# vpc-ccg/tksm

Measured on AMD Instinct MI355X. Metric: sequenced reads/s, higher is better.
Workload: dtype u8; 1 GPU; Bulk molecules, Badread error+qual model (nanopore2020, identity 84,99,5.5), 24 x 128 Mb random genome, FASTQ; kind=bulk, mean_len=1000, length_distribution=normal(1000, 200), compute_qual=True, contexts_in_flight_per_gpu=3

## Files before the change

### __graft_entry__.py

```python
import os
import subprocess
import sys

ROOT = os.path.dirname(os.path.abspath(__file__))


LLVM_BIN = "/opt/rocm/lib/llvm/bin"
NO_SPILL = ("k_alnf", "k_loop", "k_loopw", "k_err", "k_emit", "k_init")
LOOP_VGPR_LIMIT = 128
NO_SPILL_MDF = ("k_noise_plan", "k_noise_fill", "k_pal_count", "k_pal_write",
                "k_mut_count", "k_mut_write")
NO_SPILL_KDE = ("k_kde_grid", "k_kde_sum", "k_kde_cv_min", "k_kde_cv_sum")
NO_SPILL_ABUND = ("k_abund_compat", "k_abund_hits", "k_abund_msum", "k_abund_mfinish", "k_abund_mtotal", "k_abund_estep")
NO_SPILL_MS = ("k_ms_expand", "k_ms_err_events", "k_ms_qs_events")


def kernel_resources(obj):
    import re
    import shutil
    import tempfile
    d = tempfile.mkdtemp(prefix="tksm_co_")
    try:
        tmp = os.path.join(d, os.path.basename(obj))
        shutil.copy(obj, tmp)
        subprocess.check_call([os.path.join(LLVM_BIN, "llvm-objdump"), "--offloading", tmp], stdout=subprocess.DEVNULL)
        cos = [f for f in os.listdir(d) if "amdgcn" in f and "gfx950" in f]
        if not cos:
            raise RuntimeError(f"{obj}: no gfx950 code object inside")
        notes = subprocess.check_output([os.path.join(LLVM_BIN, "llvm-readelf"), "--notes", os.path.join(d, cos[0])], text=True)
    finally:
        shutil.rmtree(d, ignore_errors=True)
    out, cur = {}, None
    for block in notes.split("  - .")[1:]:
        f = dict(re.findall(r"^\s*\.?([a-z_]+):\s+(\S+)\s*$", "." + block, re.M))
        if "name" in f and "vgpr_count" in f:
            out[f["name"]] = {k: int(v) for k, v in f.items() if v.isdigit()}
    return out


def check_no_spills():
    guarded, missing = {}, []
    for obj, names in (("kernels.o", NO_SPILL), ("mdf_kernels.o", NO_SPILL_MDF), ("kde_kernels.o", NO_SPILL_KDE),
                       ("abund_kernels.o", NO_SPILL_ABUND), ("ms_kernels.o", NO_SPILL_MS)):
        res = kernel_resources(os.path.join(ROOT, "tksm_amd", "csrc", "_build", obj))
        found = {n: r for n, r in res.items() if any(f"{len(k)}{k}" in n for k in names)}
        missing += [k for k in names if not any(f"{len(k)}{k}" in n for n in found)]
        guarded.update(found)
    if missing:
        raise RuntimeError(f"spill gate: kernels {missing} not found in the code object (renamed?)")
    bad = {n: r for n, r in guarded.items() if r.get("vgpr_spill_count", 0) or r.get("private_segment_fixed_size", 0)}
    if bad:
        raise RuntimeError("spill gate: scratch spills in " + "; ".join(
            f"{n}: {r.get('vgpr_spill_count')} VGPRs spilled, {r.get('private_segment_fixed_size')} B scratch" for n, r in bad.items()))
    return guarded


def build():
    subprocess.check_call(["make", "-s", "-j8", "-C", os.path.join(ROOT, "tksm_amd", "csrc")])
    guarded = check_no_spills()
    loop = [r for n, r in guarded.items() if "6k_loopE" in n]
    if len(loop) != 1 or loop[0]["vgpr_count"] > LOOP_VGPR_LIMIT:
        raise RuntimeError(f"k_loop: {[r['vgpr_count'] for r in loop]} VGPRs, the limit is {LOOP_VGPR_LIMIT}")
    print(f"k_loop: {loop[0]['vgpr_count']} VGPRs (limit {LOOP_VGPR_LIMIT}), no scratch; LDS per wave 256 B x fragment words per lane "
          f"(at most 64: 16 KB) + the 4 KB bounds table of the first thresholds")
    subprocess.check_call(["make", "-s", "-C", os.path.join(ROOT, "oracle")])
    sys.path.insert(0, ROOT)
    import tksm_amd
    from tksm_amd import _lib
    lib = _lib.load()
    missing = [s for s in _lib.SYMBOLS if not hasattr(lib, s)]
    if missing:
        raise RuntimeError(f"libtksmseq.so lacks symbols: {missing}")


def smoke():
    sys.path.insert(0, ROOT)
    sys.path.insert(0, os.path.join(ROOT, "oracle"))
    import numpy as np
    import pyoracle as po
    from tksm_amd.sequence import Sequencer
    models = os.path.join(ROOT, "tksm_amd", "models", "badread")
    err, qs = os.path.join(models, "nanopore2020.error.gz"), os.path.join(models, "nanopore2020.qscore.gz")
    rs = np.random.RandomState(3)
    ref = {f"c{i}": rs.choice(np.frombuffer(b"ACGT", np.uint8), 50_000).tobytes().decode() for i in range(2)}
    s = Sequencer(0)
    for k, v in ref.items():
        s.add_contig(k, v)
    s.set_identity(84.0, 99.0, 5.5)
    s.load_error_model(err)
    s.load_qscore_model(qs)
    mols = []
    for i in range(16):
        st = int(rs.randint(0, 40_000))
        mols.append((f"m{i}", [(f"c{i % 2}", st, st + 400 + 20 * i, "+-"[i % 2], "3T" if i % 3 == 0 else ""),
                               ("ACGTTTTT", 0, 8, "+", "")]))
    text = "".join(f"+{m}\t1\t\n" + "".join(f"{c}\t{a}\t{b}\t{st}\t{md}\n" for c, a, b, st, md in ivs) for m, ivs in mols)
    b = s.batch_from_mdf(text)
    recs = s.run(b, target="badread", fastq=True, compute_qual=True, seed=9).records()
    perfect = s.run(b, target="perfect", fastq=True, seed=9).records()
    ident = po.Identities(84.0, 5.5, 99.0)
    em, qm = po.ErrorModel(err), po.QScoreModel(qs)
    for i, (mid, ivs) in enumerate(mols):
        raw = po.splice(ref, ivs)
        want, _ = po.badread_record(True, 9, i, raw, ident, em, qm, True, mid)
        assert recs[i] == want, f"badread record {i} differs from the oracle"
        assert perfect[i] == po.perfect_record(True, 9, i, raw, mid), f"perfect record {i} differs from the oracle"
    s.close()
    print("smoke ok: 16 badread + 16 perfect records bit-exact vs the CPU oracle")


if __name__ == "__main__":
    build()
    if len(sys.argv) > 1 and sys.argv[1] == "smoke":
        smoke()
```

### tksm_amd/csrc/ctx.h

```cpp
#pragma once
#include <hip/hip_runtime.h>
#include <chrono>

#include <algorithm>
#include <cstdint>
#include <cstdio>
#include <cstdlib>
#include <map>
#include <memory>
#include <mutex>
#include <string>
#include <unordered_map>
#include <vector>

#include "../../include/tksmseq.h"
#include "abund_kernels.h"
#include "host.h"
#include "kernels.h"
#include "tsb_host.h"

using namespace tkh;

#define HIPCHK(ctx, call)                                                                         \
    do {                                                                                          \
// ... 151 lines not shown
        if (was_owned) release(); else { p = nullptr; cap = 0; }
        p = np; cap = ncap; owned = true; dev = ndev;
        return hipSuccess;
    }
    template <class T> T* as() const { return (T*)p; }
};

struct TmpBuf : DevBuf {
    explicit TmpBuf(hipStream_t s) { pooled = true; pool_stream = s; }
};

struct PinnedBuf {
    void* p = nullptr;
    size_t cap = 0;
    hipError_t ensure(size_t bytes) {
        if (bytes <= cap) return hipSuccess;
        release();
        const hipError_t e = hipHostMalloc(&p, bytes * 2, hipHostMallocDefault);
        if (e != hipSuccess) { p = nullptr; return e; }
        cap = bytes * 2;
        if (Poison::get().on) Poison::get().fill_host(p, cap);
        return hipSuccess;
    }
    void release() { if (p) (void)hipHostFree(p); p = nullptr; cap = 0; }
    ~PinnedBuf() { release(); }
    template <class T> T* as() const { return (T*)p; }
};

struct HelperStream {
    hipStream_t stream = nullptr;
    hipEvent_t start = nullptr, done = nullptr;
    bool used = false;
    hipError_t fork_from(hipStream_t main) {
        hipError_t e = stream ? hipSuccess : hipStreamCreateWithFlags(&stream, hipStreamNonBlocking);
        for (hipEvent_t* ev : {&start, &done}) if (e == hipSuccess && !*ev) e = hipEventCreateWithFlags(ev, hipEventDisableTiming);
        if (e == hipSuccess) e = hipEventRecord(start, main);
        if (e == hipSuccess) e = hipStreamWaitEvent(stream, start, 0);
        return e;
    }
    hipError_t launched() { const hipError_t e = hipEventRecord(done, stream); used = used || e == hipSuccess; return e; }
    hipError_t wait_done() { return hipEventSynchronize(done); }
    hipError_t join_into(hipStream_t main) { return hipStreamWaitEvent(main, done, 0); }
    bool idle() const { return !used || hipEventQuery(done) == hipSuccess; }
    hipError_t synchronize() { return stream ? hipStreamSynchronize(stream) : hipSuccess; }
    ~HelperStream() {
        if (stream) { (void)hipStreamSynchronize(stream); (void)hipStreamDestroy(stream); }
        for (hipEvent_t ev : {start, done}) if (ev) (void)hipEventDestroy(ev);
    }
};

enum RunDiag {
    DIAG_ROUNDS, DIAG_EXACT_KERNEL_READS, DIAG_PREDICTED_STRAGGLERS, DIAG_JOBS_14_ROW_ROUNDS, DIAG_JOBS_REDONE_FULL_WIDTH, DIAG_FALLBACKS,
    DIAG_FALLBACK_REASONS, DIAG_FALLBACKS_QSCORE_JOBS, DIAG_FALLBACKS_LIST_PASS, DIAG_JOBS_ALL_ROUNDS, DIAG_BAND_EXITS,
    DIAG_WORDS = 16
};

struct tksmseq_batch {
    uint64_t n_reads = 0, n_intervals = 0, n_mods = 0, n_literals = 0;
    DevBuf reads, intervals, mods, literals, litpool, ids, idpool;
    tksmseq_batch() { for (DevBuf* b : {&reads, &intervals, &mods, &literals, &litpool, &ids, &idpool, &d_dup, &d_order, &d_tail}) b->pooled = true; }
    std::vector<uint32_t> h_dup;
    DevBuf d_dup;
    std::vector<uint32_t> h_comments;
    std::vector<char> h_comment_pool;
    std::vector<uint32_t> raw_len;
    std::vector<uint32_t> order;
    DevBuf d_order;
    uint32_t max_raw = 0;
    uint64_t total_raw = 0;
    std::vector<uint32_t> splice_len;
    DevBuf d_tail;
    bool tail_on = false;
    uint64_t tail_key[4] = {};
    int cache_k = -1, cache_num = 0, cache_den = 0, cache_add = 0;
    uint64_t cache_scratch = 0;
};

struct tksmseq_ctx : ContigLookup {
    int device = 0;
    int n_cus = 256;
    hipStream_t stream = nullptr;
    static constexpr int N_SIDE = 4, SIDE_WAVES = 512;
    HelperStream side[N_SIDE];
    HelperStream early;
    uint32_t early_tail = 1024;
    DevBuf f_early;
    bool own_stream = false;
    std::string err;

    std::vector<std::string> contig_names;
    std::unordered_map<std::string, int> contig_index;
    std::vector<uint64_t> contigs;
    uint64_t total_alloc = 0;
    uint64_t total_bases = 0;
    uint32_t pool_blocks = 0;
    std::vector<uint8_t> contig_declared; uint32_t n_declared = 0;
    uint64_t ref_version = 0, wgs_version = ~0ull;
    DevBuf d_wgs_sofar, d_wgs_nameoff, d_wgs_namelen, d_wgs_names;
    DevBuf d_packed, d_blocktab, d_pool, d_contigs, d_stage;
    std::shared_ptr<const tsb::Transcripts> tsb;
    uint64_t tsb_dev_serial = 0, tsb_ref_version = ~0ull;
    DevBuf d_tsb_first, d_tsb_exons, d_tsb_lits, d_tsb_litpool;
    uint64_t tsb_n_lits = 0, tsb_lit_bytes = 0;
    float tsb_plan_ms = 0.f, tsb_write_ms = 0.f;
    uint64_t mut_serial = 0, mut_ref_version = ~0ull;
    DevBuf d_mut_refctg, d_mut_nameoff, d_mut_names, d_mut_delfirst, d_mut_ptfirst, d_mut_delfrom, d_mut_delto, d_mut_ptpos, d_mut_ptinfo, d_mut_insent, d_mut_inspool;
// ... 62 lines not shown
```

### tksm_amd/csrc/kernels.h

```cpp
#pragma once
#include <hip/hip_runtime.h>
#include <stdint.h>

namespace tk {

constexpr uint32_t NO_BLOCK = 0xFFFFFFFFu;
constexpr int BLOCK_SHIFT = 12;
constexpr int WAVES_PER_WG = 4;

struct RefView {
    const uint32_t* packed;
    const uint32_t* blocktab;
    const uint8_t* pool;
    const uint64_t* contigs;
    uint32_t n_contigs;
};

struct BatchView {
    const uint32_t* reads;
    const uint32_t* intervals;
    const uint32_t* mods;
    const uint64_t* literals;
    const uint8_t* litpool;
    const uint32_t* ids;
// ... 72 lines not shown
    unsigned long long* work_counter;
    int32_t* istats;
    double* dstats;
    uint8_t* full_pool; unsigned long long full_pool_bytes; unsigned long long* full_pool_used;
    const uint32_t* tail_len;
    const TailChain* tail_chain;
    uint8_t* big_scratch; size_t big_per_wave; unsigned long long* big_trace;
    const uint32_t* read_list;
    uint64_t n_work;
};

struct ReadState {
    double errors, target, est;
    int32_t change_count;
    uint32_t n_base, aln_no;
    int16_t resume_src, resume_j;
    uint8_t stage;
    uint8_t pending, slow, early;
    int32_t st_draws, st_aligns;
    uint32_t job;
    int32_t raw_len;
    uint32_t res_mt, res_cols, res_fail, pad3;
};

struct RangeGeo {
    uint64_t trace_off;
    uint64_t jc_off;
    uint64_t popd_off;
    uint64_t unused;
    uint32_t tstride;
    uint32_t cw;
    uint32_t ncap;
    uint32_t pad;
};

enum Counter {
    CNT_JOBS = 0,
    CNT_DEFERRED = 1,
    CNT_SLOW = 2,
    CNT_FULL_ROWS = 3,
    CNT_EXIT = 4,
    CNT_REDO_JOBS = 8,
    CNT_REDO_WAVES = 9,
    CNT_REDO_LIST = 10,
    CNT_FAIL = 12,
    CNT_FAIL_OR = 13,
    CNT_FAIL_LAST = 14,
    CNT_FAIL_NM = 15,
    CNT_FAIL_REASON = 16,
    CNT_FAIL_QJOB = 24,
    CNT_FAIL_LIST = 25,
    CNT_EARLY_SLOW = 26,
    CNT_EARLY = 27,
    CNT_WORDS = 32
};
enum ExitCause { EXIT_BAND_LOOP = 0, EXIT_SHIFT_LOOP = 1, EXIT_SHIFT_ERR = 2, EXIT_BAND_ERR = 3 };
enum FailBit { FAIL_QUEUE = 0, FAIL_NOROW = 1, FAIL_SHIFT31 = 3, FAIL_SHIFT14 = 4, FAIL_END_CELL = 5, FAIL_WALK = 6 };

struct FastBuffers {
    ReadState* state;
    const uint32_t* row64;
    uint8_t* st_frag;
    uint16_t* st_nb;
    unsigned long long* st_fplanes;
    uint32_t* st_frag2;
    uint32_t* job_meta;
    uint8_t* job_popd;
    void* trace;
    uint32_t* redo_list;
    void* trace_full;
    uint32_t full_rows, full_tg;
    uint32_t full_cl;
    uint32_t* counters;
    uint32_t* job_cnt;
    uint32_t rs, n_ranges;
    const uint32_t* prev_meta; const uint8_t* prev_popd;
    const uint32_t* prefix;
    const uint32_t* base_cur; const uint32_t* base_prev;
    const RangeGeo* geo_cur; const RangeGeo* geo_prev;
    uint32_t* slow_list;
    uint32_t* early_hist;
    uint2* early_list;
    uint32_t* early_slow;
    uint2* defer_list;
    uint32_t* defer_cnt;
    int defer_len;
};

hipError_t launch_pack(const uint8_t* ascii, uint64_t n, uint64_t gstart, uint32_t* packed, uint32_t* blockflag,
                       hipStream_t s);
hipError_t launch_fill_pool(const uint8_t* ascii, uint64_t n, uint64_t gstart, const uint32_t* blocktab,
                            uint8_t* pool, hipStream_t s);
hipError_t launch_read_lengths(const BatchView& b, const RefView& r, int k, int cap_num, int cap_den, int cap_add,
                               const uint32_t* tail_len, uint32_t* raw_len, uint64_t* slot_cap, uint32_t* status, hipStream_t s);
hipError_t launch_tail_lengths(const BatchView& B, const RefView& R, const TailView& T, uint64_t seed, uint64_t first_read,
                               uint64_t stride, uint32_t* tail_len, hipStream_t s);
hipError_t launch_simulate(const BatchView& b, const RefView& r, const ErrModelView& em, const QsModelView& qm,
                           const IdentView& im, const SimParams& p, const SimBuffers& o, int n_wgs,
                           int waves_per_wg, hipStream_t s);
size_t simulate_big_bytes(int lcap, int ncap);
hipError_t launch_simulate_big(const BatchView& b, const RefView& r, const ErrModelView& em, const QsModelView& qm,
                               const IdentView& im, const SimParams& p, const SimBuffers& o, int n_waves, hipStream_t s);
hipError_t launch_init(const BatchView& b, const RefView& r, const ErrModelView& em, const IdentView& im, const SimParams& p,
                       const SimBuffers& o, const FastBuffers& fb, int waves_per_wg, hipStream_t s);
int err_lds_bytes(int lcap, int ncap, int waves_per_wg, bool state_in_hbm);
int loop_lds_words(int lcap);
// ... 34 lines not shown
```

### tksm_amd/csrc/kernels.hip

```cpp
#include "kernels.h"
#include "loop_filter.h"
#include <type_traits>

namespace tk {

#define DEV __device__ __forceinline__

constexpr int BIG = 1 << 28;
DEV bool is_inf(int v) { return v >= (1 << 27); }

struct Ph4 { uint32_t x, y, z, w; };
enum { ST_ID = 0, ST_PAD = 1, ST_IDENT = 2, ST_DRAW = 3, ST_ALNPOS = 4, ST_QUAL = 5, ST_TAIL = 6 };

DEV Ph4 philox(uint64_t seed, uint64_t read, uint32_t stream, uint32_t n) {
    uint32_t c0 = (uint32_t)read, c1 = (uint32_t)(read >> 32), c2 = stream, c3 = n;
    uint32_t k0 = (uint32_t)seed, k1 = (uint32_t)(seed >> 32);
#pragma unroll
    for (int r = 0; r < 10; r++) {
        const unsigned long long p0 = (unsigned long long)0xD2511F53u * c0, p1 = (unsigned long long)0xCD9E8D57u * c2;
        const uint32_t h0 = (uint32_t)(p0 >> 32), l0 = (uint32_t)p0, h1 = (uint32_t)(p1 >> 32), l1 = (uint32_t)p1;
        uint32_t n0 = h1 ^ c1 ^ k0, n2 = h0 ^ c3 ^ k1;
        c0 = n0; c1 = l1; c2 = n2; c3 = l0;
        k0 += 0x9E3779B9u; k1 += 0xBB67AE85u;
    }
    return Ph4{c0, c1, c2, c3};
}

DEV uint8_t base_char(int code) { return (uint8_t)((0x54474341u >> (8 * (code & 3))) & 0xff); }
DEV int code_of(uint8_t c) { return c == 'A' ? 0 : c == 'C' ? 1 : c == 'G' ? 2 : c == 'T' ? 3 : -1; }
DEV uint8_t upper(uint8_t c) { return (c >= 'a' && c <= 'z') ? (uint8_t)(c - 32) : c; }
DEV uint8_t comp(uint8_t c) {
    return c == 'A' ? 'T' : c == 'C' ? 'G' : c == 'G' ? 'C' : c == 'T' ? 'A' : c;
}

template <int CTRL, int ROW_MASK> DEV int dpp_mov(int old, int src) { return __builtin_amdgcn_update_dpp(old, src, CTRL, ROW_MASK, 0xf, false); }
constexpr int DPP_WAVE_SHL1 = 0x130, DPP_WAVE_SHR1 = 0x138;
#define TKSM_DPP_SCAN(OP, IDENT, x)                         \
    x = OP(x, dpp_mov<0x111, 0xf>(IDENT, x));               \
    x = OP(x, dpp_mov<0x112, 0xf>(IDENT, x));               \
    x = OP(x, dpp_mov<0x114, 0xf>(IDENT, x));               \
    x = OP(x, dpp_mov<0x118, 0xf>(IDENT, x));               \
    x = OP(x, dpp_mov<0x142, 0xa>(IDENT, x));               \
    x = OP(x, dpp_mov<0x143, 0xc>(IDENT, x));
DEV int scan_min_incl(int x, int) { TKSM_DPP_SCAN(min, 0x7fffffff, x) return x; }
DEV int scan_max_incl(int x, int) { TKSM_DPP_SCAN(max, (int)0x80000000, x) return x; }
DEV int add_i32(int a, int b) { return a + b; }
DEV int scan_add_incl(int x, int) { TKSM_DPP_SCAN(add_i32, 0, x) return x; }
DEV uint32_t scan_umax_incl(uint32_t x) {
#define TKSM_UMAX_STEP(C, R) x = max(x, (uint32_t)dpp_mov<C, R>(0, (int)x));
    TKSM_UMAX_STEP(0x111, 0xf) TKSM_UMAX_STEP(0x112, 0xf) TKSM_UMAX_STEP(0x114, 0xf) TKSM_UMAX_STEP(0x118, 0xf) TKSM_UMAX_STEP(0x142, 0xa) TKSM_UMAX_STEP(0x143, 0xc)
#undef TKSM_UMAX_STEP
    return x;
}
DEV int prefix_small(int v, int& total) {
// ... 1610 lines not shown
        uint32_t lo2 = c0, hi2 = c1 - 1;
        while (lo2 < hi2) { const uint32_t mid = (lo2 + hi2 + 1) >> 1; if (FB.prefix[mid] <= target) lo2 = mid; else hi2 = mid - 1; }
        const uint32_t pjob = FB.base_prev[lo2] + (target - FB.prefix[lo2]);
        r = (uint64_t)__builtin_amdgcn_readfirstlane((int)FB.prev_meta[4ull * pjob]) & 0xffffffffull;
        pos = lo2 * FB.rs;
    }
    ReadState S = FB.state[r];
    if (S.stage == 2 || S.slow) return;
    if (S.stage == 0) return;
    uint16_t* gnb = nb_row(FB, r);
    const int per_wave = STATE_IN_HBM ? lds_ncap + 128 : lds_lcap * 3 + lds_ncap + 128;
    uint8_t* lds_wave = lds_raw + (size_t)wave * per_wave;
    uint8_t* frag = STATE_IN_HBM ? frag_row(FB, r) : lds_wave;
    uint16_t* nb = STATE_IN_HBM ? gnb : reinterpret_cast<uint16_t*>(lds_wave + lds_lcap);
    uint8_t* aux = STATE_IN_HBM ? lds_wave : lds_wave + 3 * (size_t)lds_lcap;
    const int k = EM.k;
    const uint64_t g = P.first_read + r * P.stride;
    const int raw_len = __builtin_amdgcn_readfirstlane(S.raw_len);
    const int L = raw_len + 2 * k;
    const uint64_t slot = O.slot_off[r];
    const int cap = __builtin_amdgcn_readfirstlane((int)((O.slot_off[r + 1] - slot) >> 1));
    uint8_t* out_seq = O.scratch + slot;
    uint8_t* out_qual = out_seq + cap;
    if (!STATE_IN_HBM) {
        const uint8_t* gfrag0 = frag_row(FB, r);
        for (int t = lane * 4; t < L; t += 256) *reinterpret_cast<uint32_t*>(frag + t) = *reinterpret_cast<const uint32_t*>(gfrag0 + t);
        for (int t = lane * 2; t < L; t += 128) *reinterpret_cast<uint32_t*>(nb + t) = *reinterpret_cast<const uint32_t*>(gnb + t);
    }
    wave_sync();
    uint32_t status = 0;
    const double frag_len = (double)L;
    const double errors = S.errors;
    const double target = S.target;
    const int change_count = __builtin_amdgcn_readfirstlane(S.change_count), st_draws = __builtin_amdgcn_readfirstlane(S.st_draws);
    int st_aligns = __builtin_amdgcn_readfirstlane(S.st_aligns);
    double identity = 1.0;

    int start_trim, end_trim;
    {
        int v1 = lane < k ? slot_len(nb[lane]) : 0, v2 = lane < k ? slot_len(nb[L - k + lane]) : 0;
        (void)prefix_small(v1, start_trim);
        (void)prefix_small(v2, end_trim);
    }
    const int jcap = min(lds_ncap, cap);
    const int m = joined_len(nb, 0, L, lane);
    int lo = start_trim, hi = end_trim == 0 ? 0 : m - end_trim;
    lo = min(lo, m); hi = max(hi, lo);
    if (m > jcap) { status |= 1; lo = hi = 0; }
    const int out_len = hi - lo;
    const bool want_q = P.compute_q && m > 0 && !(status & 1);
    if (want_q) {
        const uint32_t mt = S.res_mt, cols = S.res_cols, fail = S.res_fail;
        if (fail) { go_slow(FB, r, lane, EXIT_BAND_ERR); return; }
        identity = cols ? (double)mt / (double)cols : 0.0;
        const uint32_t rc1 = pos / FB.rs;
        const uint8_t* gp = FB.prev_popd + FB.geo_prev[rc1].popd_off + (size_t)(S.job - FB.base_prev[rc1]) * FB.geo_prev[rc1].ncap;
        wave_sync();
        uint8_t* popd = aux + 16;
        for (int t = lane; t < m; t += 64) popd[t] = gp[t];
        wave_sync();
        const int margins = (QM.kmer_size - 1) / 2;
        const uint32_t hmask = (uint32_t)QM.n_slots - 1u;
        for (int i2 = lo + lane; i2 < hi; i2 += 64) {
#ifdef TKSM_ABLATE
            if (P.ablate == 40) { out_qual[i2 - lo] = 40; continue; }
#endif
            const int d = max(0, max(margins - i2, i2 + margins - (m - 1)));
            int row = -1; uint32_t roff = 0, rcnt = 0;
            auto probe = [&](uint64_t key) {
                uint32_t sl = (uint32_t)qs_hash(key) & hmask;
#ifdef TKSM_ABLATE
                if (P.ablate == 41) { row = (int)(sl & 1023u); roff = 0u; rcnt = 1u; return; }
#endif
                for (;;) {
                    const uint4 e = QM.ent[sl];
                    const uint64_t kk = ((uint64_t)e.y << 32) | e.x;
                    if (kk == key) { row = (int)sl; roff = e.z; rcnt = e.w; break; }
                    if (kk == 0) break;
                    sl = (sl + 1) & hmask;
                }
            };
            if (margins <= 4) {
                const int ob = 16 + i2 - 4, sh = ob & 3;
                const uint32_t* aw = reinterpret_cast<const uint32_t*>(aux) + (ob >> 2);
                const uint32_t w0 = aw[0], w1 = aw[1], w2 = aw[2];
                const uint32_t b0 = __builtin_amdgcn_alignbyte(w1, w0, sh), b1 = __builtin_amdgcn_alignbyte(w2, w1, sh), b2 = w2 >> (8 * sh);
                auto byte_at = [&](int j) -> uint32_t { return j < 4 ? (b0 >> (8 * j)) & 255u : j < 8 ? (b1 >> (8 * (j - 4))) & 255u : b2 & 255u; };
                uint64_t K[5]; int ln[5];
                K[0] = byte_at(4) & 3u; ln[0] = 1;
#pragma unroll
                for (int h = 1; h <= 4; h++) {
                    const uint32_t bl = byte_at(4 - h);
                    const int ddl = (int)(bl >> 2), ddr = (int)(byte_at(3 + h) >> 2);
                    ln[h] = ln[h - 1] + 2 + ddl + ddr;
                    const bool fits = ln[h] <= 29;
                    const int sl_ = fits ? 2 * (1 + ddl) : 0, sr_ = fits ? 2 * (1 + ddl + ln[h - 1]) : 0, so_ = fits ? 2 * (ln[h] - 1) : 0;
                    const int dl2 = fits ? 2 * ddl : 0, dr2 = fits ? 2 * ddr : 0;
                    K[h] = (uint64_t)(bl & 3u) | (((1ull << dl2) - 1ull) << 2) | (K[h - 1] << sl_) | (((1ull << dr2) - 1ull) << sr_) |
                           ((uint64_t)(byte_at(4 + h) & 3u) << so_);
                }
                const int hmax = margins - d;
                bool pend = true;
#pragma unroll
                for (int h = 4; h >= 0; h--) {
                    const bool tryit = pend && h <= hmax;
                    if (__ballot(tryit) == 0ull) continue;
                    if (tryit && ln[h] <= 29) { probe(K[h] | ((uint64_t)ln[h] << 58)); pend = row < 0; }
#ifdef TKSM_ABLATE
                    if (P.ablate == 44) { if (row < 0) row = (int)(K[h] & 1023u); pend = false; }
                    if (P.ablate == 45 && h == 3) { if (row < 0) row = (int)(K[h] & 1023u); pend = false; }
#endif
                }
            } else {
                int s0 = i2 - margins + d, e0 = i2 + margins - d;
                for (;;) {
                    uint64_t key = 0; int len = 0; bool ok = true;
                    for (int x2 = s0; x2 <= e0; x2++) {
                        if (x2 > s0) {
                            const int dd = popd[x2 - 1] >> 2;
                            if (len + dd > 29) { ok = false; break; }
                            key |= ((1ull << (2 * dd)) - 1ull) << (2 * len); len += dd;
                        }
                        if (len >= 29) { ok = false; break; }
                        key |= (uint64_t)(popd[x2] & 3) << (2 * len); len++;
                    }
                    if (ok) probe(key | ((uint64_t)len << 58));
                    if (row >= 0 || s0 == e0) break;
                    s0++; e0--;
                }
            }
            uint8_t q = 0;
#ifdef TKSM_ABLATE
            if (P.ablate == 42) { out_qual[i2 - lo] = (uint8_t)(33 + (row & 31)); continue; }
            if (P.ablate == 43 && row >= 0) {
                const uint32_t w = (uint32_t)i2 * 2654435761u;
                const uint32_t a2 = QM.guide[(size_t)row * 64 + (w >> 26)] & 0x7fu;
                out_qual[i2 - lo] = (uint8_t)(33 + QM.pairs[roff + min(a2, rcnt - 1u)].y); continue;
            }
#endif
            if (row >= 0) {
                const uint32_t w = philox(P.seed, g, ST_QUAL, (uint32_t)i2).x;
                uint32_t a2 = QM.guide[(size_t)row * 64 + (w >> 26)];
                if (QM.guide_direct && (a2 & 0x80u)) q = (uint8_t)(a2 & 0x7fu);
                else {
                    uint2 pr = QM.pairs[roff + a2];
                    while (a2 + 1 < rcnt && !(w < pr.x)) { a2++; pr = QM.pairs[roff + a2]; }
                    q = (uint8_t)pr.y;
                }
            }
            out_qual[i2 - lo] = (uint8_t)(q + 33);
        }
    } else {
        identity = 1.0 - errors / frag_len;
    }
    join_out(frag, nb, L, out_seq, lo, hi, lane);
    if (P.quirk_perfect) identity = 1.0;
    finish_read(B, P, O, r, P.quirk_perfect ? out_len : raw_len, out_len, identity, status, st_draws, change_count, st_aligns, L, m,
                start_trim, end_trim, errors, target, lane);
    if (lane == 0) FB.state[r].stage = 2;
}

__global__ void k_collect_unfinished(FastBuffers FB, uint64_t n_reads) {
    const uint64_t r = (uint64_t)blockIdx.x * blockDim.x + threadIdx.x;
    if (r >= n_reads) return;
    ReadState S = FB.state[r];
    if (S.stage != 2 && !S.slow) {
        FB.state[r].slow = 1;
        const uint32_t idx = atomicAdd(&FB.counters[CNT_SLOW], 1u);
        FB.slow_list[idx] = (uint32_t)r;
    }
}

DEV uint32_t range_of_job(const FastBuffers& FB, uint32_t job0) {
    uint32_t rng = 0, hi2 = FB.n_ranges - 1;
    while (rng < hi2) { const uint32_t mid = (rng + hi2 + 1) >> 1; if (FB.base_cur[mid] <= job0) rng = mid; else hi2 = mid - 1; }
    return rng;
}
__global__ __launch_bounds__(64) void k_qjobs(FastBuffers FB, int k, uint32_t count) {
    const int lane = threadIdx.x;
    const uint32_t widx = blockIdx.x * 64u + (uint32_t)lane;
    bool need = widx < count;
    uint32_t r = 0, rc = 0, job = 0;
    if (need) { const uint2 e = FB.defer_list[widx]; r = e.x; rc = e.y; }
    need = need && FB.state[r].stage == 3 && !FB.state[r].slow;
    const bool mine = need;
    unsigned long long todo = __ballot(need);
    while (todo) {
        const int leader = __builtin_ctzll(todo);
        const uint32_t lrc = (uint32_t)__shfl((int)rc, leader, 64);
        const unsigned long long grp = __ballot(need && rc == lrc);
        uint32_t base = 0;
        if (lane == leader) base = FB.base_cur[lrc] + atomicAdd(&FB.job_cnt[lrc * 32u], (uint32_t)__popcll(grp));
        base = (uint32_t)__shfl((int)base, leader, 64);
        if (need && rc == lrc) { job = base + (uint32_t)__popcll(grp & ((1ull << lane) - 1ull)); need = false; }
        todo &= ~grp;
    }
    if (mine) {
        ReadState* sp = FB.state + r;
        const uint32_t L = (uint32_t)(sp->raw_len + 2 * k);
        *reinterpret_cast<uint4*>(FB.job_meta + 4ull * job) = make_uint4(r, 0u, L | 0x80000000u, 0u);
        sp->resume_src = -1; sp->pending = 1; sp->stage = 1; sp->job = job;
    }
}

DEV int wave_max(int v) {
#pragma unroll
    for (int o = 32; o > 0; o >>= 1) v = max(v, __shfl_xor(v, o, 64));
    return v;
// ... 1009 lines not shown
```

### tksm_amd/csrc/run.cpp

```cpp
#include "../../include/tksmseq.h"

#include <hip/hip_runtime.h>

#include <algorithm>
#include <cstdio>
#include <cstring>
#include <cstdlib>
#include <string>

#include "ctx.h"

#define TRY(call) do { const int rc_ = (call); if (rc_ != TKSMSEQ_OK) return rc_; } while (0)

static tk::BatchView batch_view(const tksmseq_batch* b) {
    return tk::BatchView{b->reads.as<uint32_t>(), b->intervals.as<uint32_t>(), b->mods.as<uint32_t>(), b->literals.as<uint64_t>(),
                         b->litpool.as<uint8_t>(), b->ids.as<uint32_t>(), b->idpool.as<uint8_t>(), b->n_reads, (uint32_t)b->n_literals};
}
static tk::RefView ref_view(const tksmseq_ctx* ctx) {
    return tk::RefView{ctx->d_packed.as<uint32_t>(), ctx->d_blocktab.as<uint32_t>(), ctx->d_pool.as<uint8_t>(),
                       ctx->d_contigs.as<uint64_t>(), (uint32_t)ctx->contig_names.size()};
}

static int apply_tail(tksmseq_ctx* ctx, tksmseq_batch* b, const tksmseq_run_params* p) {
    const bool want = p->mode == TKSMSEQ_MODE_BADREAD && ctx->tail.enabled && b->n_reads > 0;
// ... 408 lines not shown
    int align(bool qround) {
        const uint32_t jobs = cnt[tk::CNT_JOBS];
        const uint32_t n_jobs = hbase_cur[FB.n_ranges - 1] + ((hcnt[(size_t)(FB.n_ranges - 1) * 32] + 63) & ~63u);
        const bool full_only = jobs <= std::min(ctx->small_aln, full_rows_fit);
        jobs_all += jobs; if (!full_only) jobs_14 += jobs;
        HIPCHK(ctx, tk::launch_alnf(pl.P, FB, pl.O, n_jobs, full_only, qround ? 1 : 0, s));
        return tick(ALN);
    }
    int rounds() {
        for (;; n_rounds++) {
            select_set(n_rounds);
            HIPCHK(ctx, tk::launch_round_reset(FB, s));
            TRY(tick(GAP));
            const bool qround = revive && pl.P.compute_q;
            const bool regular = !revive && !revived;
            TRY(revive ? launch_revive() : revived ? launch_last_visits() : launch_loops());
            TRY(tick(regular ? JOB : OTHER));
            TRY(exchange());
            TRY(flush_side());
            if (cnt[tk::CNT_JOBS] == 0) {
                TRY(join_early());
                if (cnt[tk::CNT_DEFERRED] == 0 || revived) break;
                revived = revive = true; n_deferred = cnt[tk::CNT_DEFERRED];
                std::vector<uint32_t> hd((size_t)FB.n_ranges * 32);
                HIPCHK(ctx, hipMemcpy(hd.data(), ctx->f_defercnt.p, hd.size() * 4, hipMemcpyDeviceToHost));
                HIPCHK(ctx, pack_ranges(hd.data(), true));
                continue;
            }
#ifdef TKSM_ABLATE
            if (pl.P.ablate >= 1 && pl.P.ablate <= 9) break;
#endif
            if (cnt[tk::CNT_JOBS] < ctx->tail_cut && cnt[tk::CNT_JOBS] * 64ull < n) {
                HIPCHK(ctx, tk::launch_collect_unfinished(FB, n, s));
                HIPCHK(ctx, hipMemcpyAsync(cnt, FB.counters, 64, hipMemcpyDeviceToHost, s));
                HIPCHK(ctx, hipStreamSynchronize(s));
                break;
            }
            if (n_rounds > 100000) { ctx->err = "internal: error loop did not terminate"; return TKSMSEQ_EDEVICE; }
            TRY(tick(GAP));
            TRY(align(qround));
            HIPCHK(ctx, pack_ranges(hcnt, false));
        }
        pl.mark("rounds done");
        return TKSMSEQ_OK;
    }
    int finish(float ms[3]) {
        uint32_t* d = ctx->last_diag;
        memset(d, 0, sizeof(ctx->last_diag));
        d[DIAG_ROUNDS] = n_rounds; d[DIAG_EXACT_KERNEL_READS] = cnt[tk::CNT_SLOW]; d[DIAG_PREDICTED_STRAGGLERS] = n_early;
        d[DIAG_JOBS_14_ROW_ROUNDS] = (uint32_t)std::min<uint64_t>(jobs_14, 0xffffffffu); d[DIAG_JOBS_REDONE_FULL_WIDTH] = cnt[tk::CNT_REDO_JOBS];
        d[DIAG_FALLBACKS] = cnt[tk::CNT_FAIL]; d[DIAG_FALLBACK_REASONS] = cnt[tk::CNT_FAIL_OR]; d[DIAG_FALLBACKS_QSCORE_JOBS] = cnt[tk::CNT_FAIL_QJOB];
        d[DIAG_FALLBACKS_LIST_PASS] = cnt[tk::CNT_FAIL_LIST]; d[DIAG_JOBS_ALL_ROUNDS] = (uint32_t)std::min<uint64_t>(jobs_all, 0xffffffffu);
        d[DIAG_BAND_EXITS] = cnt[tk::CNT_EXIT + tk::EXIT_BAND_LOOP] + cnt[tk::CNT_EXIT + tk::EXIT_BAND_ERR];
        if (pl.vlevel) {
            uint32_t cc[tk::CNT_WORDS];
            HIPCHK(ctx, hipMemcpy(cc, FB.counters, sizeof(cc), hipMemcpyDeviceToHost));
            const uint32_t *ex = cc + tk::CNT_EXIT, *why = cc + tk::CNT_FAIL_REASON;
            fprintf(stderr, "[tksmseq] this thread so far: %u device allocations, %.3f s in hipMalloc\n", alloc_calls(), alloc_seconds());
            fprintf(stderr, "[tksmseq] reads %llu rounds %u slow-path reads %u (band exit %u/%u, shift %u/%u), full-width redo: %u jobs in %u waves; predicted stragglers on their own stream: %u\n",
                    (unsigned long long)n, n_rounds, cnt[tk::CNT_SLOW], ex[tk::EXIT_BAND_LOOP], ex[tk::EXIT_BAND_ERR], ex[tk::EXIT_SHIFT_LOOP], ex[tk::EXIT_SHIFT_ERR], cc[tk::CNT_REDO_JOBS], cc[tk::CNT_REDO_WAVES], n_early);
            fprintf(stderr, "[tksmseq] fused alignment failures: %u, reasons or-ed 0x%x, last 0x%x (n %u, m %u)\n", cc[tk::CNT_FAIL], cc[tk::CNT_FAIL_OR], cc[tk::CNT_FAIL_LAST], cc[tk::CNT_FAIL_NM] & 0xffffu, cc[tk::CNT_FAIL_NM] >> 16);
            fprintf(stderr, "[tksmseq]   per reason: queue / reservoir overflow %u no pool rows %u - shift>31 %u shift>14 %u end cell %u walk %u | q-score jobs %u, list pass %u\n", why[tk::FAIL_QUEUE], why[tk::FAIL_NOROW], why[tk::FAIL_SHIFT31], why[tk::FAIL_SHIFT14], why[tk::FAIL_END_CELL], why[tk::FAIL_WALK], cc[tk::CNT_FAIL_QJOB], cc[tk::CNT_FAIL_LIST]);
        }
        for (HelperStream& h : ctx->side) if (h.used) HIPCHK(ctx, h.join_into(s));
        if (cnt[tk::CNT_SLOW] > n_side) {
            pl.O.read_list = ctx->f_slow.as<uint32_t>() + n_side; pl.O.n_work = cnt[tk::CNT_SLOW] - n_side;
            const uint64_t want = (pl.O.n_work + pl.wpw - 1) / pl.wpw;
            TRY(tick(GAP));
            HIPCHK(ctx, tk::launch_simulate(pl.B, pl.R, pl.EM, pl.QM, pl.IM, pl.P, pl.O, (int)std::max<uint64_t>(1, std::min<uint64_t>(want, (uint64_t)pl.n_wgs)), pl.wpw, s));
            TRY(tick(OTHER));
        }
        if (ctx->timing) {
            HIPCHK(ctx, hipStreamSynchronize(s));
            for (size_t i = 1; i < kinds.size(); i++) {
                float t = 0; (void)hipEventElapsedTime(&t, ctx->evpool[i - 1], ctx->evpool[i]);
                if (kinds[i] >= LOOP) ms[kinds[i] - LOOP] += t;
            }
        }
        return TKSMSEQ_OK;
    }
};

static int rerun_in_hbm(const RunPlan& pl, const std::vector<uint32_t>& st) {
    tksmseq_ctx* ctx = pl.ctx;
    hipStream_t s = ctx->stream;
    std::vector<uint32_t> big;
    for (uint64_t i = 0; i < pl.n; i++) if (st[i] & 8) big.push_back((uint32_t)i);
    const int n_waves = (int)std::min<size_t>(big.size(), 64);
    const size_t per_wave = tk::simulate_big_bytes(pl.lcap, pl.ncap);
    HIPCHK(ctx, ctx->w_biglist.ensure(big.size() * 4 + 16));
    HIPCHK(ctx, ctx->w_bigscratch.ensure(per_wave * n_waves + 64));
    HIPCHK(ctx, ctx->w_bigtrace.ensure((size_t)n_waves * 2 * (pl.ncap + 2) * 8 + 64));
    HIPCHK(ctx, hipMemcpyAsync(ctx->w_biglist.p, big.data(), big.size() * 4, hipMemcpyHostToDevice, s));
    HIPCHK(ctx, hipMemsetAsync(ctx->w_counter.p, 0, 8, s));
    tk::SimBuffers O3 = pl.O;
    O3.read_list = ctx->w_biglist.as<uint32_t>(); O3.n_work = big.size();
    O3.work_counter = ctx->w_counter.as<unsigned long long>();
    O3.big_scratch = ctx->w_bigscratch.as<uint8_t>(); O3.big_per_wave = per_wave; O3.big_trace = ctx->w_bigtrace.as<unsigned long long>();
    HIPCHK(ctx, tk::launch_simulate_big(pl.B, pl.R, pl.EM, pl.QM, pl.IM, pl.P, O3, n_waves, s));
    if (pl.vlevel) fprintf(stderr, "[tksmseq] %zu molecules beyond the LDS-resident limit took the exact kernel with HBM working sets\n", big.size());
    return TKSMSEQ_OK;
}

static int check_status(const RunPlan& pl, int pass, bool* again, bool* overflow) {
    tksmseq_ctx* ctx = pl.ctx;
    const uint64_t n = pl.n;
// ... 131 lines not shown
```

### tksm_amd/sequence.py

```python
import ctypes as C

import numpy as np

from . import _lib as L

BGZF_EOF = bytes.fromhex("1f8b08040000000000ff0600424302001b0003000000000000000000")


class TksmSeqError(RuntimeError):
    def __init__(self, code, msg):
        super().__init__(f"tksmseq error {code}: {msg}")
        self.code = code


class Batch:
    def __init__(self, seq, handle):
        self._seq, self._h = seq, handle
        n, ni, nm = C.c_uint64(), C.c_uint64(), C.c_uint64()
        seq._lib.tksmseq_batch_info(handle, C.byref(n), C.byref(ni), C.byref(nm))
        self.n_reads, self.n_intervals, self.n_mods = n.value, ni.value, nm.value

    def free(self):
        if self._h:
            self._seq._lib.tksmseq_batch_free(self._seq._ctx, self._h)
# ... 514 lines not shown
        t, n = C.c_void_p(), C.c_uint64()
        self._chk(self._lib.tksmseq_batch_to_mdf_text(self._ctx, batch._h, C.byref(t), C.byref(n)))
        try:
            return C.string_at(t, n.value).decode()
        finally:
            self._lib.tksmseq_text_free(t)

    def run(self, batch, target="badread", fastq=True, compute_qual=True, seed=42, first_read_index=0, stride=1,
            collect_stats=False, perfect_of_badread=False):
        p = L.RunParams(seed, first_read_index, stride, L.MODE_BADREAD if target == "badread" else L.MODE_PERFECT,
                        1 if fastq else 0, 1 if compute_qual else 0, 1 if collect_stats else 0,
                        1 if perfect_of_badread else 0, 0)
        r = L.Result()
        self._chk(self._lib.tksmseq_run(self._ctx, batch._h, C.byref(p), C.byref(r)))
        return RunResult(self, r)

    def mdf_to_seq(self, molecules, target="perfect", **kw):
        lines = []
        for mid, intervals in molecules:
            lines.append(f"+{mid}\t1\t\n")
            for chrom, start, end, strand, mods in intervals:
                lines.append(f"{chrom}\t{start}\t{end}\t{strand}\t{mods}\n")
        b = self.batch_from_mdf("".join(lines))
        try:
            return self.run(b, target=target, **kw).records()
        finally:
            b.free()

    def _gzip_fetch(self, g, with_info):
        out = np.empty(g.bytes, np.uint8)
        self._chk(self._lib.tksmseq_gzip_download_range(self._ctx, out.ctypes.data, 0, g.bytes, 0))
        if not with_info:
            return out.tobytes()
        off = np.empty(g.n_members + 1, np.uint64)
        self._chk(self._lib.tksmseq_gzip_download_offsets(self._ctx, off.ctypes.data))
        return out.tobytes(), off, g.device_ms

    def gzip_device(self, ptr, nbytes, format=L.GZIP_RAW, with_info=False):
        fmt = {"raw": L.GZIP_RAW, "fasta": L.GZIP_FASTA, "fastq": L.GZIP_FASTQ}.get(format, format)
        g = L.GzipResult()
        self._chk(self._lib.tksmseq_gzip_device(self._ctx, C.c_void_p(ptr) if ptr else None, nbytes, fmt, C.byref(g)))
        return self._gzip_fetch(g, with_info)

    def set_host_threads(self, n):
        self._chk(self._lib.tksmseq_set_host_threads(self._ctx, int(n)))

    def set_timing(self, on=True):
        self._chk(self._lib.tksmseq_set_timing(self._ctx, 1 if on else 0))

    def run_diagnostics(self):
        out = (C.c_uint32 * 16)()
        self._chk(self._lib.tksmseq_run_diagnostics(self._ctx, out))
        keys = ("rounds", "exact_kernel_reads", "predicted_stragglers", "jobs_14_row_rounds", "jobs_redone_full_width", "fallbacks",
                "fallback_reasons", "fallbacks_qscore_jobs", "fallbacks_list_pass", "jobs_all_rounds", "band_exits")
        return {k: int(out[i]) for i, k in enumerate(keys)}

    def set_output_buffer(self, ptr, capacity):
        self._chk(self._lib.tksmseq_set_output_buffer(self._ctx, C.c_void_p(ptr) if ptr else None, capacity))

    def synchronize(self):
        self._chk(self._lib.tksmseq_synchronize(self._ctx))

    def interleave_records(self, streams, offsets, n_per_rank, dst_ptr, dst_capacity):
        n = len(streams)
        sp = (C.c_void_p * n)(*[C.c_void_p(s) for s in streams])
        op = (C.c_void_p * n)(*[C.c_void_p(o) for o in offsets])
        npr = (C.c_uint64 * n)(*n_per_rank)
        out = C.c_uint64()
        self._chk(self._lib.tksmseq_interleave_records(self._ctx, n, sp, op, npr, C.c_void_p(dst_ptr), dst_capacity,
                                                       C.byref(out)))
        return out.value


def random_wgs_main(argv):
    lib = L.load()
    arr = (C.c_char_p * len(argv))(*[a.encode() for a in argv])
    return lib.tksmseq_random_wgs_main(len(argv), arr)


def transcribe_main(argv):
    lib = L.load()
    arr = (C.c_char_p * len(argv))(*[a.encode() for a in argv])
    return lib.tksmseq_transcribe_main(len(argv), arr)


def sequence_main(argv):
    lib = L.load()
    arr = (C.c_char_p * len(argv))(*[a.encode() for a in argv])
    return lib.tksmseq_sequence_main(len(argv), arr)


def build_tail_model(mapped, unmapped, lx, ly, begin, trans, bandwidth, path, device=0):
    import json
    mapped = np.asarray(mapped, np.float64).ravel(); unmapped = np.asarray(unmapped, np.float64).ravel()
    lx = np.asarray(lx, np.float64).ravel(); ly = np.asarray(ly, np.float64).ravel()
    trans = np.asarray(trans, np.float64); begin = np.asarray(begin, np.float64).ravel()
    if len(mapped) != len(unmapped) or len(mapped) == 0:
        raise ValueError("tail model: mapped and unmapped must be non-empty and of one length")
    if len(lx) != len(ly):
        raise ValueError("tail model: lx and ly must have the same length (the reference's sampler reads grid rows by ly)")
    if trans.shape != (4, 4) or begin.shape != (4,):
        raise ValueError("tail model: begin must hold 4 weights, trans 4 x 4")
    s = Sequencer(device)
    try:
        grid = s.kde_grid(np.stack([mapped, unmapped], axis=1), lx, ly, bandwidth)
    finally:
        s.close()
# ... 6 lines not shown
```

Measured before the change: 15.66 million reads/s.

## Build qscore k-mer keys from a packed LDS op stream with prefix offsets

For the quality-score pass, each wave now packs the alignment op sequence into a 2-bit token stream in LDS, using a wave prefix scan for offsets. Each position's centred window key for sizes 4..1 then becomes a single bit-slice of that stream, replacing the per-position byte-walk key construction. The old per-position path is kept as a fallback when the stream does not fit in LDS or the state lives in HBM. The change also moves join_out ahead of the quality pass and adds diagnostic counters, which cost extra atomics in the hot loop.

```diff
diff --git a/__graft_entry__.py b/__graft_entry__.py
--- a/__graft_entry__.py
+++ b/__graft_entry__.py
@@ -8,6 +8,7 @@
 LLVM_BIN = "/opt/rocm/lib/llvm/bin"
 NO_SPILL = ("k_alnf", "k_loop", "k_loopw", "k_err", "k_emit", "k_init")
 LOOP_VGPR_LIMIT = 128
+ERR_VGPR_LIMIT = 64
 NO_SPILL_MDF = ("k_noise_plan", "k_noise_fill", "k_pal_count", "k_pal_write",
                 "k_mut_count", "k_mut_write")
 NO_SPILL_KDE = ("k_kde_grid", "k_kde_sum", "k_kde_cv_min", "k_kde_cv_sum")
@@ -63,6 +64,10 @@
         raise RuntimeError(f"k_loop: {[r['vgpr_count'] for r in loop]} VGPRs, the limit is {LOOP_VGPR_LIMIT}")
     print(f"k_loop: {loop[0]['vgpr_count']} VGPRs (limit {LOOP_VGPR_LIMIT}), no scratch; LDS per wave 256 B x fragment words per lane "
           f"(at most 64: 16 KB) + the 4 KB bounds table of the first thresholds")
+    err = {("<true>" if "ILb1E" in n else "<false>"): r["vgpr_count"] for n, r in guarded.items() if "5k_errI" in n}
+    if len(err) != 2 or max(err.values()) > ERR_VGPR_LIMIT:
+        raise RuntimeError(f"k_err: {err} VGPRs, the limit is {ERR_VGPR_LIMIT}")
+    print(f"k_err: {err['<false>']} / {err['<true>']} VGPRs (state in LDS / in HBM; limit {ERR_VGPR_LIMIT}), no scratch")
     subprocess.check_call(["make", "-s", "-C", os.path.join(ROOT, "oracle")])
     sys.path.insert(0, ROOT)
     import tksm_amd
diff --git a/tksm_amd/csrc/ctx.h b/tksm_amd/csrc/ctx.h
--- a/tksm_amd/csrc/ctx.h
+++ b/tksm_amd/csrc/ctx.h
@@ -227,6 +227,7 @@
 enum RunDiag {
     DIAG_ROUNDS, DIAG_EXACT_KERNEL_READS, DIAG_PREDICTED_STRAGGLERS, DIAG_JOBS_14_ROW_ROUNDS, DIAG_JOBS_REDONE_FULL_WIDTH, DIAG_FALLBACKS,
     DIAG_FALLBACK_REASONS, DIAG_FALLBACKS_QSCORE_JOBS, DIAG_FALLBACKS_LIST_PASS, DIAG_JOBS_ALL_ROUNDS, DIAG_BAND_EXITS,
+    DIAG_QS_KEYS_PER_POSITION, DIAG_QS_GAPS_29, DIAG_QS_WINDOWS_29, DIAG_QS_WINDOWS_30,
     DIAG_WORDS = 16
 };
 
diff --git a/tksm_amd/csrc/kernels.h b/tksm_amd/csrc/kernels.h
--- a/tksm_amd/csrc/kernels.h
+++ b/tksm_amd/csrc/kernels.h
@@ -148,6 +148,10 @@
     CNT_FAIL_LIST = 25,
     CNT_EARLY_SLOW = 26,
     CNT_EARLY = 27,
+    CNT_QS_PERPOS = 28,
+    CNT_QS_GAP29 = 29,
+    CNT_QS_LEN29 = 30,
+    CNT_QS_LEN30 = 31,
     CNT_WORDS = 32
 };
 enum ExitCause { EXIT_BAND_LOOP = 0, EXIT_SHIFT_LOOP = 1, EXIT_SHIFT_ERR = 2, EXIT_BAND_ERR = 3 };
diff --git a/tksm_amd/csrc/kernels.hip b/tksm_amd/csrc/kernels.hip
--- a/tksm_amd/csrc/kernels.hip
+++ b/tksm_amd/csrc/kernels.hip
@@ -1,5 +1,6 @@
 #include "kernels.h"
 #include "loop_filter.h"
+#include "qs_keys.h"
 #include <type_traits>
 
 namespace tk {
@@ -1716,6 +1717,7 @@
     if (want_q) {
         const uint32_t mt = S.res_mt, cols = S.res_cols, fail = S.res_fail;
         if (fail) { go_slow(FB, r, lane, EXIT_BAND_ERR); return; }
+        join_out(frag, nb, L, out_seq, lo, hi, lane);
         identity = cols ? (double)mt / (double)cols : 0.0;
         const uint32_t rc1 = pos / FB.rs;
         const uint8_t* gp = FB.prev_popd + FB.geo_prev[rc1].popd_off + (size_t)(S.job - FB.base_prev[rc1]) * FB.geo_prev[rc1].ncap;
@@ -1725,25 +1727,98 @@
         wave_sync();
         const int margins = (QM.kmer_size - 1) / 2;
         const uint32_t hmask = (uint32_t)QM.n_slots - 1u;
+        int row = -1; uint32_t roff = 0, rcnt = 0;
+        auto probe = [&](uint64_t key) {
+            uint32_t sl = (uint32_t)qs_hash(key) & hmask;
+#ifdef TKSM_ABLATE
+            if (P.ablate == 41) { row = (int)(sl & 1023u); roff = 0u; rcnt = 1u; return; }
+#endif
+            for (;;) {
+                const uint4 e = QM.ent[sl];
+                const uint64_t kk = ((uint64_t)e.y << 32) | e.x;
+                if (kk == key) { row = (int)sl; roff = e.z; rcnt = e.w; break; }
+                if (kk == 0) break;
+                sl = (sl + 1) & hmask;
+            }
+        };
+        auto draw_q = [&](int i2) {
+            uint8_t q = 0;
+            if (row >= 0) {
+                const uint32_t w = philox(P.seed, g, ST_QUAL, (uint32_t)i2).x;
+                uint32_t a2 = QM.guide[(size_t)row * 64 + (w >> 26)];
+                if (QM.guide_direct && (a2 & 0x80u)) q = (uint8_t)(a2 & 0x7fu);
+                else {
+                    uint2 pr = QM.pairs[roff + a2];
+                    while (a2 + 1 < rcnt && !(w < pr.x)) { a2++; pr = QM.pairs[roff + a2]; }
+                    q = (uint8_t)pr.y;
+                }
+            }
+            out_qual[i2 - lo] = (uint8_t)(q + 33);
+        };
+        bool use_stream = false;
+        const uint32_t nw = tkqk::qs_stream_words(cols);
+        if constexpr (!STATE_IN_HBM) use_stream = margins <= 4 && cols >= (uint32_t)m && cols < 65536u && (int)(nw * 4u) + 2 * m <= 3 * lds_lcap;
+#ifdef TKSM_ABLATE
+        if (P.ablate >= 40 && P.ablate <= 46) use_stream = false;
+#endif
+        if constexpr (!STATE_IN_HBM) { if (!use_stream && margins <= 4 && lane == 0) atomicAdd(&FB.counters[CNT_QS_PERPOS], 1u); }
+        if (use_stream) {
+            uint32_t* strm = reinterpret_cast<uint32_t*>(lds_wave);
+            uint16_t* offs = reinterpret_cast<uint16_t*>(strm + nw);
+            for (uint32_t t = (uint32_t)lane; t < nw; t += 64) strm[t] = 0u;
+            wave_sync();
+            int base = 0;
+            for (int xb = 0; xb < m; xb += 64) {
+                const int x = xb + lane;
+                const uint32_t b = x < m ? popd[x] : 0u;
+                const int tl = x < m ? tkqk::qs_token_units(b) : 0;
+                const int incl = scan_add_incl(tl, lane);
+                const int off = base + incl - tl;
+                base += __builtin_amdgcn_readlane(incl, 63);
+                if (x < m) offs[x] = (uint16_t)off;
+                if (x < m && (b >> 2) >= (uint32_t)tkqk::QS_GAP_MAX) atomicAdd(&FB.counters[CNT_QS_GAP29], 1u);
+                const uint64_t tok = x < m ? tkqk::qs_token(b) : 0ull;
+                if (tok) {
+                    const uint32_t w = (uint32_t)off >> 4, sh = (2u * (uint32_t)off) & 31u;
+                    const uint32_t t0 = lo32(tok) << sh, t1 = sh ? alignbit(hi32(tok), lo32(tok), 32u - sh) : hi32(tok);
+                    const uint32_t t2 = sh ? hi32(tok) >> (32u - sh) : 0u;
+                    if (t0 && w < nw) atomicOr(&strm[w], t0);
+                    if (t1 && w + 1 < nw) atomicOr(&strm[w + 1], t1);
+                    if (t2 && w + 2 < nw) atomicOr(&strm[w + 2], t2);
+                }
+            }
+            wave_sync();
+            for (int i2 = lo + lane; i2 < hi; i2 += 64) {
+                const int d = max(0, max(margins - i2, i2 + margins - (m - 1)));
+                const int hmax = margins - d;
+                row = -1; roff = 0u; rcnt = 0u;
+                bool pend = true;
+#pragma unroll
+                for (int h = 4; h >= 1; h--) {
+                    const bool tryit = pend && h <= hmax;
+                    if (__ballot(tryit) == 0ull) continue;
+                    if (tryit) {
+                        const uint32_t o0 = offs[i2 - h];
+                        const int len = (int)(offs[i2 + h] - o0) + 1;
+                        uint64_t key;
+                        if (tkqk::qs_key_slice(strm, o0, len, key)) { probe(key); pend = row < 0; }
+                        if ((uint32_t)(len - tkqk::QS_KEY_MAX_OPS) < 2u)
+                            atomicAdd(&FB.counters[len == tkqk::QS_KEY_MAX_OPS ? CNT_QS_LEN29 : CNT_QS_LEN30], 1u);
+                    }
+                }
+                if (__ballot(pend) != 0ull) {
+                    if (pend) probe((uint64_t)(popd[i2] & 3u) | (1ull << 58));
+                }
+                draw_q(i2);
+            }
+        }
+        else
         for (int i2 = lo + lane; i2 < hi; i2 += 64) {
 #ifdef TKSM_ABLATE
             if (P.ablate == 40) { out_qual[i2 - lo] = 40; continue; }
 #endif
             const int d = max(0, max(margins - i2, i2 + margins - (m - 1)));
-            int row = -1; uint32_t roff = 0, rcnt = 0;
-            auto probe = [&](uint64_t key) {
-                uint32_t sl = (uint32_t)qs_hash(key) & hmask;
-#ifdef TKSM_ABLATE
-                if (P.ablate == 41) { row = (int)(sl & 1023u); roff = 0u; rcnt = 1u; return; }
-#endif
-                for (;;) {
-                    const uint4 e = QM.ent[sl];
-                    const uint64_t kk = ((uint64_t)e.y << 32) | e.x;
-                    if (kk == key) { row = (int)sl; roff = e.z; rcnt = e.w; break; }
-                    if (kk == 0) break;
-                    sl = (sl + 1) & hmask;
-                }
-            };
+            row = -1; roff = 0u; rcnt = 0u;
             if (margins <= 4) {
                 const int ob = 16 + i2 - 4, sh = ob & 3;
                 const uint32_t* aw = reinterpret_cast<const uint32_t*>(aux) + (ob >> 2);
@@ -1752,6 +1827,14 @@
                 auto byte_at = [&](int j) -> uint32_t { return j < 4 ? (b0 >> (8 * j)) & 255u : j < 8 ? (b1 >> (8 * (j - 4))) & 255u : b2 & 255u; };
                 uint64_t K[5]; int ln[5];
                 K[0] = byte_at(4) & 3u; ln[0] = 1;
+#ifdef TKSM_ABLATE
+                const bool no_keys = P.ablate == 46;
+                if (no_keys) {
+#pragma unroll
+                    for (int h = 1; h <= 4; h++) { K[h] = ((((uint64_t)b1 << 32) | b0) ^ ((uint64_t)b2 << 50)) & ((1ull << 58) - 1ull); ln[h] = 9; }
+                }
+                else
+#endif
 #pragma unroll
                 for (int h = 1; h <= 4; h++) {
                     const uint32_t bl = byte_at(4 - h);
@@ -1771,7 +1854,7 @@
                     if (__ballot(tryit) == 0ull) continue;
                     if (tryit && ln[h] <= 29) { probe(K[h] | ((uint64_t)ln[h] << 58)); pend = row < 0; }
 #ifdef TKSM_ABLATE
-                    if (P.ablate == 44) { if (row < 0) row = (int)(K[h] & 1023u); pend = false; }
+                    if (P.ablate == 44 || no_keys) { if (row < 0) row = (int)(K[h] & 1023u); pend = false; }
                     if (P.ablate == 45 && h == 3) { if (row < 0) row = (int)(K[h] & 1023u); pend = false; }
 #endif
                 }
@@ -1793,7 +1876,6 @@
                     s0++; e0--;
                 }
             }
-            uint8_t q = 0;
 #ifdef TKSM_ABLATE
             if (P.ablate == 42) { out_qual[i2 - lo] = (uint8_t)(33 + (row & 31)); continue; }
             if (P.ablate == 43 && row >= 0) {
@@ -1802,22 +1884,12 @@
                 out_qual[i2 - lo] = (uint8_t)(33 + QM.pairs[roff + min(a2, rcnt - 1u)].y); continue;
             }
 #endif
-            if (row >= 0) {
-                const uint32_t w = philox(P.seed, g, ST_QUAL, (uint32_t)i2).x;
-                uint32_t a2 = QM.guide[(size_t)row * 64 + (w >> 26)];
-                if (QM.guide_direct && (a2 & 0x80u)) q = (uint8_t)(a2 & 0x7fu);
-                else {
-                    uint2 pr = QM.pairs[roff + a2];
-                    while (a2 + 1 < rcnt && !(w < pr.x)) { a2++; pr = QM.pairs[roff + a2]; }
-                    q = (uint8_t)pr.y;
-                }
-            }
-            out_qual[i2 - lo] = (uint8_t)(q + 33);
+            draw_q(i2);
         }
     } else {
         identity = 1.0 - errors / frag_len;
-    }
-    join_out(frag, nb, L, out_seq, lo, hi, lane);
+        join_out(frag, nb, L, out_seq, lo, hi, lane);
+    }
     if (P.quirk_perfect) identity = 1.0;
     finish_read(B, P, O, r, P.quirk_perfect ? out_len : raw_len, out_len, identity, status, st_draws, change_count, st_aligns, L, m,
                 start_trim, end_trim, errors, target, lane);
diff --git a/tksm_amd/csrc/qs_keys.h b/tksm_amd/csrc/qs_keys.h
--- /dev/null
+++ b/tksm_amd/csrc/qs_keys.h
@@ -0,0 +1,75 @@
+#pragma once
+#include <stddef.h>
+#include <stdint.h>
+
+#if defined(__HIPCC__)
+#define TKQK_HD __host__ __device__ inline
+#else
+#define TKQK_HD inline
+#endif
+
+namespace tkqk {
+
+constexpr int QS_KEY_MAX_OPS = 29;
+constexpr int QS_GAP_MAX = 29;
+constexpr int QS_STREAM_PAD_WORDS = 3;
+
+TKQK_HD int qs_token_units(uint32_t b) { const int dd = (int)(b >> 2); return 1 + (dd < QS_GAP_MAX ? dd : QS_GAP_MAX); }
+
+TKQK_HD uint64_t qs_token(uint32_t b) {
+    const int g = qs_token_units(b) - 1;
+    return (uint64_t)(b & 3u) | (((1ull << (2 * g)) - 1ull) << 2);
+}
+
+TKQK_HD uint32_t qs_stream_words(uint32_t units) { return (2u * units + 31u) / 32u + (uint32_t)QS_STREAM_PAD_WORDS; }
+
+TKQK_HD uint64_t qs_stream_bits(const uint32_t* words, uint32_t off) {
+    const uint32_t w = off >> 4, s = (2u * off) & 31u;
+    const uint32_t a0 = words[w], a1 = words[w + 1], a2 = words[w + 2];
+#if defined(__HIP_DEVICE_COMPILE__)
+    return ((uint64_t)__builtin_amdgcn_alignbit(a2, a1, s) << 32) | __builtin_amdgcn_alignbit(a1, a0, s);
+#else
+    const uint64_t lo = ((uint64_t)a1 << 32) | a0, hi = ((uint64_t)a2 << 32) | a1;
+    return s ? ((lo >> s) & 0xffffffffull) | ((hi >> s) << 32) : lo;
+#endif
+}
+
+TKQK_HD bool qs_key_slice(const uint32_t* words, uint32_t off, int len, uint64_t& key) {
+    if (len > QS_KEY_MAX_OPS) return false;
+    key = (qs_stream_bits(words, off) & ((1ull << (2 * len)) - 1ull)) | ((uint64_t)len << 58);
+    return true;
+}
+
+inline void qs_stream_pack(const uint8_t* ops, int m, uint32_t* words, uint32_t* off) {
+    uint32_t u = 0;
+    for (int x = 0; x < m; x++) { off[x] = u; u += (uint32_t)qs_token_units(ops[x]); }
+    off[m] = u;
+    const uint32_t nw = qs_stream_words(u);
+    for (uint32_t w = 0; w < nw; w++) words[w] = 0;
+    for (int x = 0; x < m; x++) {
+        const uint64_t t = qs_token(ops[x]);
+        const uint32_t w = off[x] >> 4, s = (2u * off[x]) & 31u;
+        words[w] |= (uint32_t)t << s;
+        words[w + 1] |= (uint32_t)(s ? t >> (32 - s) : t >> 32);
+        if (s) words[w + 2] |= (uint32_t)(t >> (64 - s));
+    }
+}
+
+inline int qs_window_units(const uint32_t* off, int s0, int e0) { return (int)(off[e0] - off[s0]) + 1; }
+
+inline bool qs_key_generic(const uint8_t* ops, int s0, int e0, uint64_t& key) {
+    uint64_t k = 0; int len = 0;
+    for (int x = s0; x <= e0; x++) {
+        if (x > s0) {
+            const int dd = ops[x - 1] >> 2;
+            if (len + dd > QS_KEY_MAX_OPS) return false;
+            k |= ((1ull << (2 * dd)) - 1ull) << (2 * len); len += dd;
+        }
+        if (len >= QS_KEY_MAX_OPS) return false;
+        k |= (uint64_t)(ops[x] & 3) << (2 * len); len++;
+    }
+    key = k | ((uint64_t)len << 58);
+    return true;
+}
+
+}
diff --git a/tksm_amd/csrc/run.cpp b/tksm_amd/csrc/run.cpp
--- a/tksm_amd/csrc/run.cpp
+++ b/tksm_amd/csrc/run.cpp
@@ -484,6 +484,8 @@
         d[DIAG_FALLBACKS] = cnt[tk::CNT_FAIL]; d[DIAG_FALLBACK_REASONS] = cnt[tk::CNT_FAIL_OR]; d[DIAG_FALLBACKS_QSCORE_JOBS] = cnt[tk::CNT_FAIL_QJOB];
         d[DIAG_FALLBACKS_LIST_PASS] = cnt[tk::CNT_FAIL_LIST]; d[DIAG_JOBS_ALL_ROUNDS] = (uint32_t)std::min<uint64_t>(jobs_all, 0xffffffffu);
         d[DIAG_BAND_EXITS] = cnt[tk::CNT_EXIT + tk::EXIT_BAND_LOOP] + cnt[tk::CNT_EXIT + tk::EXIT_BAND_ERR];
+        d[DIAG_QS_KEYS_PER_POSITION] = cnt[tk::CNT_QS_PERPOS]; d[DIAG_QS_GAPS_29] = cnt[tk::CNT_QS_GAP29];
+        d[DIAG_QS_WINDOWS_29] = cnt[tk::CNT_QS_LEN29]; d[DIAG_QS_WINDOWS_30] = cnt[tk::CNT_QS_LEN30];
         if (pl.vlevel) {
             uint32_t cc[tk::CNT_WORDS];
             HIPCHK(ctx, hipMemcpy(cc, FB.counters, sizeof(cc), hipMemcpyDeviceToHost));
diff --git a/tksm_amd/sequence.py b/tksm_amd/sequence.py
--- a/tksm_amd/sequence.py
+++ b/tksm_amd/sequence.py
@@ -590,7 +590,8 @@
         out = (C.c_uint32 * 16)()
         self._chk(self._lib.tksmseq_run_diagnostics(self._ctx, out))
         keys = ("rounds", "exact_kernel_reads", "predicted_stragglers", "jobs_14_row_rounds", "jobs_redone_full_width", "fallbacks",
-                "fallback_reasons", "fallbacks_qscore_jobs", "fallbacks_list_pass", "jobs_all_rounds", "band_exits")
+                "fallback_reasons", "fallbacks_qscore_jobs", "fallbacks_list_pass", "jobs_all_rounds", "band_exits",
+                "qs_keys_per_position", "qs_gaps_29", "qs_windows_29", "qs_windows_30")
         return {k: int(out[i]) for i, k in enumerate(keys)}
 
     def set_output_buffer(self, ptr, capacity):
```

After: 15.49 million reads/s. 1.1% lower.
